# dhamm97/pycsou

Measured on AMD Instinct MI355X. Metric: PDS iters/sec on 4096² TV-deconv; achieved HBM GB/s vs roofline at 1/2/4/8 GPU, higher is better.
Workload: dtype f32

## Files before the change

include/pycsou_hip.h:

```cpp
#ifndef PYCSOU_HIP_H
#define PYCSOU_HIP_H

#include <stdint.h>
#include <hip/hip_runtime_api.h>

#ifdef __cplusplus
extern "C" {
#endif

enum { PCS_F32 = 0, PCS_F64 = 1 };
enum { PCS_OK = 0, PCS_EINVAL = -1, PCS_ELAUNCH = -2, PCS_EUNSUPPORTED = -3 };
enum { PCS_FORWARD = 0, PCS_BACKWARD = 1, PCS_CENTERED = 2 };
enum { PCS_H_L1 = 0, PCS_H_L21 = 1 };
enum { PCS_G_NULL = 0, PCS_G_NONNEG = 1, PCS_G_SEGMENT = 2 };
enum { PCS_F_NULL = 0, PCS_F_DENOISE = 1, PCS_F_SEPCONV = 2, PCS_F_GRADBUF = 3, PCS_F_CONV2D = 4, PCS_F_CONV0 = 5 };
enum { PCS_K_GRAD_FORWARD = 0, PCS_K_GRAD_BACKWARD = 1, PCS_K_GRAD_CENTERED = 2, PCS_K_LAPLACIAN = 3 };

int pcs_abi_version(void);


int pcs_deriv1_fwd(int dtype, const void* x, void* out, int ndim, const int64_t* dims, int axis, double step,
                   int kind, int edge, hipStream_t stream);
int pcs_deriv1_adj(int dtype, const void* y, void* out, int ndim, const int64_t* dims, int axis, double step,
                   int kind, int edge, hipStream_t stream);
// ... 127 lines not shown
  PCS_PATH_SMARCH_NX = 6,
  PCS_PATH_NM64 = 7,
  PCS_PATH_CONV2D = 8
};
int pcs_pds2d_path(const pcs_pds2d_args* a);
int pcs_pds2d_ntaps_len(int half);

int pcs_pds2d_halo_x(int half);
int64_t pcs_pds2d_nblocks(const pcs_pds2d_args* a);
int64_t pcs_pds2d_ws_bytes(const pcs_pds2d_args* a);
int pcs_pds2d_step(const pcs_pds2d_args* a, hipStream_t stream);
int64_t pcs_pds2d_nblocks_bands(const pcs_pds2d_args* a, int64_t ra0, int64_t rb0, int64_t ra1, int64_t rb1);
int pcs_pds2d_step_bands(const pcs_pds2d_args* a, int64_t ra0, int64_t rb0, int64_t ra1, int64_t rb1,
                         hipStream_t stream);
int pcs_pds2d_run(const pcs_pds2d_args* a, int64_t n, hipStream_t stream);

typedef struct {
  int dtype, kkind, fkind, hkind, gkind, edge;
  int64_t n0, n1;
  double tau, sigma, rho, lam, step0, step1, w0, w1, seg_a, seg_b;
  const void* x; void* xn; const void* z; void* zn; const void* g;
  double* partials;
  void* ctrl;
  double* hist;
  void* ws;
} pcs_pds2d_stencil_args;
int64_t pcs_pds2d_stencil_nblocks(const pcs_pds2d_stencil_args* a);
int64_t pcs_pds2d_stencil_ws_bytes(const pcs_pds2d_stencil_args* a);
int pcs_pds2d_stencil_step(const pcs_pds2d_stencil_args* a, hipStream_t stream);
int pcs_pds2d_stencil_run(const pcs_pds2d_stencil_args* a, int64_t n, hipStream_t stream);
// ... 97 lines not shown
```

pycsou_amd/_lib.py:

```python

import ctypes
import os

import torch

_HERE = os.path.dirname(os.path.abspath(__file__))
LIB_PATH = os.environ.get('PCS_LIB_PATH') or os.path.join(_HERE, 'lib', 'libpycsou_hip.so')

PCS_F32, PCS_F64 = 0, 1
PCS_FORWARD, PCS_BACKWARD, PCS_CENTERED = 0, 1, 2
PCS_H_L1, PCS_H_L21 = 0, 1
PCS_K_GRAD_FORWARD, PCS_K_GRAD_BACKWARD, PCS_K_GRAD_CENTERED, PCS_K_LAPLACIAN = 0, 1, 2, 3
PCS_G_NULL, PCS_G_NONNEG, PCS_G_SEGMENT = 0, 1, 2
PCS_APGD_G_L1 = 3
PCS_F_NULL, PCS_F_DENOISE, PCS_F_SEPCONV, PCS_F_GRADBUF, PCS_F_CONV2D, PCS_F_CONV0 = 0, 1, 2, 3, 4, 5
PCS_M_NONE, PCS_M_L1LOSS = 0, 1
(PCS_PATH_TILE, PCS_PATH_MARCH, PCS_PATH_NMARCH, PCS_PATH_PT, PCS_PATH_SMARCH, PCS_PATH_SMARCH_NX, PCS_PATH_NM64,
 PCS_PATH_CONV2D) = range(1, 9)
PCS_PATH_FUSED_NORMAL = (PCS_PATH_NMARCH, PCS_PATH_NM64)
KINDS = {'forward': PCS_FORWARD, 'backward': PCS_BACKWARD, 'centered': PCS_CENTERED}

_c_int, _c_i64, _c_dbl, _vp = ctypes.c_int, ctypes.c_int64, ctypes.c_double, ctypes.c_void_p
_pi64 = ctypes.POINTER(ctypes.c_int64)
_pdbl = ctypes.POINTER(ctypes.c_double)
# ... 98 lines not shown
    'pcs_apgd_step': (_c_int, [_c_int, _vp, _vp, _vp, _vp, _vp, _c_i64, _c_dbl, _c_dbl, _c_int, _c_dbl, _c_dbl,
                                _c_dbl, _vp, _vp, _vp]),
    'pcs_pds2d_halo_x': (_c_int, [_c_int]),
    'pcs_pds2d_ntaps_len': (_c_int, [_c_int]),
    'pcs_pds2d_nblocks': (_c_i64, [ctypes.POINTER(PdsArgs)]),
    'pcs_pds2d_ws_bytes': (_c_i64, [ctypes.POINTER(PdsArgs)]),
    'pcs_pds2d_step': (_c_int, [ctypes.POINTER(PdsArgs), _vp]),
    'pcs_fftconv2d_grid': (_c_i64, [_c_i64, _c_int]),
    'pcs_fftconv2d_create': (_c_int, [_c_int, _c_i64, _c_i64, _pdbl, _c_int, _c_int, _c_int, _c_int,
                                      ctypes.POINTER(_vp)]),
    'pcs_fftconv2d_apply': (_c_int, [_vp, _vp, _vp, _c_int, _vp, _c_dbl, _vp]),
    'pcs_fftconv2d_destroy': (_c_int, [_vp]),
    'pcs_pds2d_supported': (_c_int, [ctypes.POINTER(PdsArgs)]),
    'pcs_pds2d_path': (_c_int, [ctypes.POINTER(PdsArgs)]),
    'pcs_pds2d_run': (_c_int, [ctypes.POINTER(PdsArgs), _c_i64, _vp]),
    'pcs_pds2d_stencil_nblocks': (_c_i64, [ctypes.POINTER(StencilArgs)]),
    'pcs_pds2d_stencil_ws_bytes': (_c_i64, [ctypes.POINTER(StencilArgs)]),
    'pcs_pds2d_stencil_step': (_c_int, [ctypes.POINTER(StencilArgs), _vp]),
    'pcs_pds2d_stencil_run': (_c_int, [ctypes.POINTER(StencilArgs), _c_i64, _vp]),
    'pcs_pds2d_nblocks_bands': (_c_i64, [ctypes.POINTER(PdsArgs), _c_i64, _c_i64, _c_i64, _c_i64]),
    'pcs_pds2d_step_bands': (_c_int, [ctypes.POINTER(PdsArgs), _c_i64, _c_i64, _c_i64, _c_i64, _vp]),
    'pcs_comm_available': (_c_int, []),
    'pcs_comm_id_bytes': (_c_int, []),
    'pcs_comm_unique_id': (_c_int, [_vp]),
    'pcs_comm_init': (_c_int, [_vp, _c_int, _c_int, ctypes.POINTER(_vp)]),
    'pcs_comm_destroy': (_c_int, [_vp]),
    'pcs_allgather_f64': (_c_int, [_vp, _c_int, _vp, _vp, _c_i64, _vp]),
    'pcs_halo_exchange': (_c_int, [_vp, _c_int, _c_int, ctypes.POINTER(HaloSet), _vp]),
    'pcs_slab2d_create': (_c_int, [ctypes.POINTER(Slab2DDesc), _vp, ctypes.POINTER(_vp)]),
    'pcs_slab2d_overlapped': (_c_int, [_vp]),
# ... 86 lines not shown
```

pycsou_amd/csrc/pds.hip:

```cpp
#include "pds_host.hpp"
#include "pds_pt.hpp"

namespace pcs {

__global__ void k_ctrl_init(Ctrl* c, int min_iter, int max_iter, double thr, int has_dual, int hist_len) {
  c->it = 0;
  c->min_iter = min_iter;
  c->max_iter = max_iter;
  c->thr = thr;
  c->has_dual = has_dual;
  c->hist_len = hist_len;
  c->pend = c->pad1 = 0;
  const double inf = __builtin_huge_val();
  c->stopped = !((0 <= min_iter) || (0 <= max_iter && inf > thr));
}

constexpr int kRedThreads = 1024;

__device__ __forceinline__ void sum_partials(const double* __restrict__ part, int64_t np, double (&v)[4]) {
  const double4* p4 = reinterpret_cast<const double4*>(part);
  double4 a[4];
#pragma unroll
  for (int u = 0; u < 4; ++u) a[u] = make_double4(0.0, 0.0, 0.0, 0.0);
  for (int64_t i = threadIdx.x; i < np; i += 4 * kRedThreads) {
// ... 114 lines not shown
                                             : (a->halo_z > a->halo_y ? a->halo_z : a->halo_y);
  if (!(a->n0 < (1LL << 30) && (a->rows + 2 * hmax) * a->n1 * 4 <= (1LL << 30))) return false;
  MarchPlan p;
  return pt_plan(a, full_bands(a), &p);
}

template <int FK, int HK>
static int launch_pt(const pcs_pds2d_args* a, RowBands rb, hipStream_t st) {
  MarchPlan p;
  if (!pt_plan(a, rb, &p)) return PCS_EINVAL;
  if (p.ntasks == 0) return PCS_OK;
  const Slab s64 = make_slab(a);
  const Slab32 s{(int)s64.n0, (int)s64.n1, (int)s64.row0, (int)s64.rows, s64.hx, s64.hy, s64.hz, s64.vec};
  const Params<float> P = make_params<float>(a);
  const float* g = FK == PCS_F_DENOISE ? (const float*)a->y : FK == PCS_F_GRADBUF ? (const float*)a->gbuf : nullptr;
  k_pds2d_pt<FK, HK><<<(unsigned)p.ntasks + fin_extra(a), 256, 0, st>>>((const float*)a->x, (float*)a->xn, (const float*)a->z,
                                                         (float*)a->zn, g, s, P, a->gkind, a->partials,
                                                         (Ctrl*)a->ctrl, a->hist, a->ws, red_out(a), p.tiles_x, p.bd,
                                                         p.ntasks);
  return launch_status();
}

static int64_t bands_nblocks(const pcs_pds2d_args* a, RowBands rb);

template <int FK>
static int launch_pt(const pcs_pds2d_args* a, RowBands rb, hipStream_t st) {
  return a->hkind == PCS_H_L21 ? launch_pt<FK, PCS_H_L21>(a, rb, st) : launch_pt<FK, PCS_H_L1>(a, rb, st);
}

static int pds2d_bands(const pcs_pds2d_args* a, RowBands rb, hipStream_t st) {
  if (use_nm64(a)) return launch_nmarch64(a, rb, st);
  if (use_smarch(a)) return a->dtype == PCS_F64 ? sm_launch<double>(a, rb, st) : sm_launch<float>(a, rb, st);
  if (use_march(a)) return launch_march(a, rb, st);
// ... 190 lines not shown

int pcs_pds2d_step(const pcs_pds2d_args* a, hipStream_t st) {
  int rc = check_args(a);
  if (rc != PCS_OK) return rc;
  if (a->fkind == PCS_F_CONV2D) {
    rc = conv2d_prepass(a, st);
    if (rc != PCS_OK) return rc;
    const pcs_pds2d_args b = step_args(a);
    return pcs_pds2d_step(&b, st);
  }
  if (a->dtype == PCS_F32) return pds2d<float>(a, st);
  if (a->dtype == PCS_F64) return pds2d<double>(a, st);
  return PCS_EINVAL;
}

int pcs_pds2d_run(const pcs_pds2d_args* a, int64_t n, hipStream_t st) {
  if (!a || n < 0 || !a->hist) return PCS_EINVAL;
  pcs_pds2d_args b = *a;
  for (int64_t i = 0; i < n; ++i) {
    if (i % 2) {
      b.x = a->xn, b.xn = const_cast<void*>(a->x), b.z = a->zn, b.zn = const_cast<void*>(a->z);
      b.zm = a->zmn, b.zmn = const_cast<void*>(a->zm);
      if (a->fin_partials) b.partials = const_cast<double*>(a->fin_partials), b.fin_partials = a->partials;
    } else {
      b.x = a->x, b.xn = a->xn, b.z = a->z, b.zn = a->zn;
      b.zm = a->zm, b.zmn = a->zmn;
      b.partials = a->partials, b.fin_partials = a->fin_partials;
    }
    const int rc = pcs_pds2d_step(&b, st);
    if (rc != PCS_OK) return rc;
  }
  return PCS_OK;
}

int64_t pcs_ctrl_bytes(void) { return 64; }

#ifdef PCS_STAMPS
int pcs_debug_stamps(void* host, int64_t bytes) {
  return hipMemcpyFromSymbol(host, HIP_SYMBOL(g_pcs_stamps), (size_t)bytes, 0, hipMemcpyDeviceToHost) == hipSuccess
             ? 0
             : PCS_ELAUNCH;
}
#endif

int pcs_ctrl_init2(void* ctrl, int min_iter, int max_iter, double thr, int has_dual, int hist_len, hipStream_t st) {
// ... 42 lines not shown
```

pycsou_amd/csrc/pds_ctrl.hpp:

```cpp
#pragma once

#include "common.hpp"

namespace pcs {

struct Ctrl {
  int32_t it, stopped, min_iter, max_iter, has_dual, hist_len;
  int32_t pend;
  int32_t pad1;
  double thr;
  double pad2;
};
static_assert(sizeof(Ctrl) == 48, "ctrl layout");

__device__ __forceinline__ void finalize_from(const double* v, Ctrl* c, double* hist) {
  const int it = c->it;
  const double inf = __builtin_huge_val();
  const double rp = (v[1] == 0.0) ? inf : sqrt(v[0]) / sqrt(v[1]);
  const double rd = (v[3] == 0.0) ? inf : sqrt(v[2]) / sqrt(v[3]);
  if (2 * it + 1 < c->hist_len) {
    hist[2 * it] = rp;
    hist[2 * it + 1] = rd;
  }
  const int nx = it + 1;
// ... 36 lines not shown
__device__ __forceinline__ bool stop_deferred(const RedOut& ro) { return PCS_DEFER_STOP && ro.sums == nullptr; }
__device__ __forceinline__ int stop_flag_early(const Ctrl* ctrl, const RedOut& ro) {
  return stop_deferred(ro) && ctrl != nullptr ? ctrl->stopped : 0;
}

__device__ __forceinline__ bool stop_requested(const Ctrl* ctrl, const RedOut& ro, int* flag) {
  if (ctrl == nullptr) return false;
  if (ro.sums == nullptr) return ctrl->stopped != 0;
  if (threadIdx.x == 0) flag[0] = __hip_atomic_load(&ctrl->stopped, __ATOMIC_RELAXED, __HIP_MEMORY_SCOPE_AGENT);
  __syncthreads();
  return flag[0] != 0;
}

constexpr int kFinBlocks = 8;
constexpr int kFinLanes = 256;
__device__ __forceinline__ int fin_shift(const RedOut& ro) { return ro.fin != nullptr ? kFinBlocks : 0; }

__device__ __forceinline__ void finalize_pending(const double* __restrict__ prev, int64_t nb, Ctrl* c, double* hist,
                                                 bool mark, double* red, int* flag) {
  const int tid = threadIdx.x;
  if (tid == 0) flag[0] = c->pend && !c->stopped;
  __syncthreads();
  if (flag[0]) {
    double v[4] = {0.0, 0.0, 0.0, 0.0};
    if (tid < kFinLanes) {
      for (int64_t j = tid; j < nb; j += kFinLanes) {
#pragma unroll
        for (int k = 0; k < 4; ++k) v[k] += prev[j * 4 + k];
      }
    }
    block_sum<4>(v, red);
    if (tid == 0) finalize_from(v, c, hist);
  }
  if (tid == 0) c->pend = mark ? 1 : 0;
}

__device__ __forceinline__ bool fin_slot(const RedOut& ro, int64_t nblocks, Ctrl* ctrl, double* hist, double* red,
                                         int* flag) {
  if (ro.fin == nullptr || blockIdx.x >= kFinBlocks) return false;
  if (blockIdx.x == 0) finalize_pending(ro.fin, nblocks, ctrl, hist, true, red, flag);
  return true;
}

#ifndef PCS_RED_ABL
#define PCS_RED_ABL 0
#endif
__device__ __forceinline__ void reduce_and_finalize(const double (&part)[4], double* __restrict__ partials,
                                                    int64_t nblocks, void* ws, Ctrl* ctrl, double* hist, int* flag,
                                                    RedOut ro = RedOut{nullptr, nullptr, 0, nullptr}) {
  if (PCS_RED_ABL & 1) return;
  const int tid = threadIdx.x;
  const int64_t b = blockIdx.x;
  const int64_t ngr = red_groups(nblocks);
  double* gsum = reinterpret_cast<double*>(ws);
  unsigned* cnt = reinterpret_cast<unsigned*>(gsum + ngr * 4);
// ... 85 lines not shown
```

pycsou_amd/csrc/pds_host.hpp:

```cpp
#pragma once

#include "pds_march.hpp"
#include "pds_nmarch.hpp"
#include "pds_smarch.hpp"

namespace pcs {

template <typename T>
struct Tile {
  static constexpr int TH = 31;
  static constexpr int NT = 256;
};
template <>
struct Tile<double> {
  static constexpr int TH = 15;
  static constexpr int NT = 256;
};

static int tier_for(int half) {
  if (half <= 3) return 3;
  if (half <= 7) return 7;
  if (half <= 11) return 11;
  if (half <= 15) return 15;
  return -1;
// ... 16 lines not shown
  P.rho = (T)a->rho;
  P.omr = (T)(1.0 - a->rho);
  const double t_h = (1.0 / a->sigma) * a->lam;
  P.t_h = (T)t_h;
  P.inv_t_h = (T)(1.0 / t_h);
  P.lam = (T)a->lam;
  P.inv_step0 = (T)(1.0 / a->step0);
  P.inv_step1 = (T)(1.0 / a->step1);
  P.unit0 = a->step0 == 1.0;
  P.unit1 = a->step1 == 1.0;
  P.seg_a = (T)a->seg_a;
  P.seg_b = (T)a->seg_b;
  return P;
}

static RedOut red_out(const pcs_pds2d_args* a) {
  return a->hist ? RedOut{nullptr, nullptr, 0, a->fin_partials}
                 : RedOut{a->sums_out, a->pre_partials, (int)a->n_pre, nullptr};
}
static unsigned fin_extra(const pcs_pds2d_args* a) {
  return a->hist && a->fin_partials ? (unsigned)kFinBlocks : 0u;
}

constexpr int kMarchNT = 256;
constexpr int kNMarchNT = 256;

struct MarchPlan {
  int tiles_x;
  Bands bd;
  int ntasks;
  StripSplit sp{-1, 0, 0, 0, {0, 0, 0}, Bands{16, 0, 0, 0, 0, 0}};
};

struct RowBands {
  int64_t ra0, rb0, ra1, rb1;
};
static RowBands full_bands(const pcs_pds2d_args* a) { return RowBands{0, a->rows, a->rows, a->rows}; }

static void plan_bands(RowBands rb, int TS, int tiles_x, int slots, int min_steps, MarchPlan* p) {
  if (rb.rb0 == rb.ra0) rb = RowBands{rb.ra1, rb.rb1, rb.rb1, rb.rb1};
  const int64_t L0 = rb.rb0 - rb.ra0, L1 = rb.rb1 - rb.ra1;
  const int64_t steps = (L0 + TS - 1) / TS + (L1 + TS - 1) / TS;
  const int64_t bands = (L0 > 0) + (L1 > 0);
  int64_t nseg = slots / tiles_x;
  const int64_t max_seg = (steps + min_steps - 1) / min_steps;
  nseg = nseg > max_seg ? max_seg : nseg;
  nseg = nseg < bands ? bands : nseg;
  nseg = nseg < 1 ? 1 : nseg;
  const int64_t seg_len = ((steps + nseg - 1) / nseg) * TS;
  const int64_t n0 = (L0 + seg_len - 1) / seg_len, n1 = (L1 + seg_len - 1) / seg_len;
  p->tiles_x = tiles_x;
  p->bd = Bands{(int)seg_len, (int)n0, (int)rb.ra0, (int)rb.rb0, (int)rb.ra1, (int)rb.rb1};
  p->ntasks = (int)(tiles_x * (n0 + n1));
}
// ... 156 lines not shown
```

pycsou_amd/csrc/pds_nm.hip:

```cpp
#include "pds_host.hpp"

namespace pcs {

template <int H>
static int march_slots() {
  static int slots = 0;
  if (slots == 0) {
    int dev = 0, cus = 0, nb = 0;
    if (hipGetDevice(&dev) != hipSuccess || hipDeviceGetAttribute(&cus, hipDeviceAttributeMultiprocessorCount, dev) !=
                                                hipSuccess || cus < 1)
      cus = 256;
    if (hipOccupancyMaxActiveBlocksPerMultiprocessor(&nb, k_pds2d_march<float, H, PCS_H_L21, kMarchNT>, kMarchNT,
                                                     0) != hipSuccess ||
        nb < 1)
      nb = 3;
    (void)hipGetLastError();
    slots = cus * nb;
  }
  return slots;
}

template <int H>
static int nmarch_slots(bool gen) {
  static int slots_f = 0, slots_g = 0;
// ... 21 lines not shown

int march_slots_h(int H) { return H == 3 ? march_slots<3>() : march_slots<7>(); }
int nmarch_slots_h(int H, bool gen) { return H == 3 ? nmarch_slots<3>(gen) : nmarch_slots<7>(gen); }

template <int H, int HK>
static int launch_march_k(const pcs_pds2d_args* a, RowBands rb, hipStream_t st) {
  MarchPlan p;
  if (!march_plan<H>(a, rb, &p)) return PCS_EINVAL;
  if (p.ntasks == 0) return PCS_OK;
  const Slab s64 = make_slab(a);
  const Slab32 s{(int)s64.n0, (int)s64.n1, (int)s64.row0, (int)s64.rows, s64.hx, s64.hy, s64.hz, s64.vec};
  const Params<float> P = make_params<float>(a);
  if (use_nmarch(a) && a->kkind != PCS_K_GRAD_FORWARD) {
    auto kern = a->kkind == PCS_K_GRAD_BACKWARD ? k_pds2d_nmarch_gen<float, H, HK, kNMarchNT, PCS_BACKWARD>
                                                : k_pds2d_nmarch_gen<float, H, HK, kNMarchNT, PCS_CENTERED>;
    kern<<<(unsigned)p.ntasks + fin_extra(a), kNMarchNT, 0, st>>>((const float*)a->x, (float*)a->xn, (const float*)a->z, (float*)a->zn,
                                                   (const float*)a->cty, (const float*)a->ntaps, s, P, a->gkind,
                                                   a->edge, a->partials, (Ctrl*)a->ctrl, a->hist, a->ws, red_out(a),
                                                   p.tiles_x, p.bd, p.ntasks);
    return launch_status();
  }
  if (use_nmarch(a)) {
    k_pds2d_nmarch<float, H, HK, kNMarchNT><<<(unsigned)p.ntasks + fin_extra(a), kNMarchNT, 0, st>>>(
        (const float*)a->x, (float*)a->xn, (const float*)a->z, (float*)a->zn, (const float*)a->cty,
        (const float*)a->ntaps, s, P, a->gkind, a->partials, (Ctrl*)a->ctrl, a->hist, a->ws, red_out(a), p.tiles_x,
        p.bd, p.ntasks);
    return launch_status();
  }
  if (a->kkind != PCS_K_GRAD_FORWARD) return PCS_EUNSUPPORTED;
  k_pds2d_march<float, H, HK, kMarchNT><<<(unsigned)p.ntasks + fin_extra(a), kMarchNT, 0, st>>>(
      (const float*)a->x, (float*)a->xn, (const float*)a->z, (float*)a->zn, (const float*)a->y,
      (const float*)a->taps0, (const float*)a->taps1, a->half, s, P, a->gkind, a->partials, (Ctrl*)a->ctrl, a->hist,
      a->ws, red_out(a), p.tiles_x, p.bd, p.ntasks);
  return launch_status();
}

template <int H>
static int launch_march_k(const pcs_pds2d_args* a, RowBands rb, hipStream_t st) {
  return a->hkind == PCS_H_L21 ? launch_march_k<H, PCS_H_L21>(a, rb, st) : launch_march_k<H, PCS_H_L1>(a, rb, st);
}

int launch_march(const pcs_pds2d_args* a, RowBands rb, hipStream_t st) {
  return tier_for(a->half) == 3 ? launch_march_k<3>(a, rb, st) : launch_march_k<7>(a, rb, st);
}

}
```

pycsou_amd/csrc/pds_nm64.hip:

```cpp
#include "pds_host.hpp"

namespace pcs {

template <int H>
struct NM64 {
  static constexpr int NT = 512, TS = 32, TO = 60, CW = 64, CC = CW / 2;
  static constexpr int NQ = 4 * H + 1;
  static constexpr int XOFF = 16, XW = CW + 2 * XOFF, XCH = XW / 2;
  static constexpr int XRING = 48, XP = XW + 2;
  static constexpr int TRING = TS + 4 * H, TMIR = 4 * H + 1, TP = CW + 2;
  static constexpr int URING = TS + 2, UP = CW + 2;
  static constexpr int ZR = TS + 2, ZCH = CC + 2;
  static constexpr int ZSL = ZR * ZCH, ZINS = (ZSL + 63) / 64;
  static constexpr int NW = 64 + 32 * H;
  static constexpr int NXL = (TS * XCH + NT - 1) / NT;
  static constexpr int O_X = 0, O_T = O_X + XRING * XP, O_U = O_T + (TRING + TMIR) * TP, O_Z = O_U + URING * UP,
                       O_W = O_Z + 2 * (ZINS * 64 * 2), SZ = O_W + NW;
  static_assert(XRING >= TS + 2 * H, "x ring holds the U rows and the PH rows of a step");
  static_assert(NT == 16 * CC && NT == TS * 16, "one PH item and one PV / U / Z item per thread");
  static __device__ __forceinline__ int xslot(int r) { return (int)((unsigned)(r + XRING * (1 << 20)) % XRING); }
  static __device__ __forceinline__ int tslot(int r) { return (int)((unsigned)(r + TRING * (1 << 20)) % TRING); }
  static __device__ __forceinline__ int uslot(int r) { return (int)((unsigned)(r + URING * (1 << 20)) % URING); }
};

// ... 420 lines not shown
    if (hipOccupancyMaxActiveBlocksPerMultiprocessor(&nb, k_pds2d_nmarch64<7, PCS_H_L21, PCS_CENTERED>, 512,
                                                     NM64<7>::SZ * sizeof(double)) != hipSuccess ||
        nb < 1)
      nb = 1;
    (void)hipGetLastError();
    slots = cus * nb;
    const char* e = getenv("PCS_NM64_SLOTS");
    if (e && atoi(e) > 0) slots = atoi(e);
  }
  return slots;
}

bool nm64_plan(const pcs_pds2d_args* a, RowBands rb, MarchPlan* p) {
  const int tiles_x = (int)((a->n1 + 59) / 60);
  if (tiles_x < 2) return false;
  if (rb.rb0 == rb.ra0) rb = RowBands{rb.ra1, rb.rb1, rb.rb1, rb.rb1};
  const int64_t L0 = rb.rb0 - rb.ra0, L1 = rb.rb1 - rb.ra1;
  const int64_t steps = (L0 + 31) / 32 + (L1 + 31) / 32;
  const int64_t bands = (L0 > 0) + (L1 > 0);
  const int64_t slots = nm64_slots();
  int64_t best = -1, seg_len = 32;
  for (int64_t nseg = bands; nseg <= steps && nseg <= 64; ++nseg) {
    const int64_t len = ((steps + nseg - 1) / nseg) * 32;
    const int64_t n = (L0 + len - 1) / len + (L1 + len - 1) / len;
    const int64_t rounds = (n * tiles_x + slots - 1) / slots;
    const int64_t cost = rounds * (len / 32 + 1);
    if (best < 0 || cost < best) {
      best = cost;
      seg_len = len;
    }
  }
  const int64_t n0s = (L0 + seg_len - 1) / seg_len, n1s = (L1 + seg_len - 1) / seg_len;
  p->tiles_x = tiles_x;
  p->bd = Bands{(int)seg_len, (int)n0s, (int)rb.ra0, (int)rb.rb0, (int)rb.ra1, (int)rb.rb1};
  p->ntasks = (int)(tiles_x * (n0s + n1s));
  return true;
}

template <int H, int HK, int KK>
static int nm64_go(const pcs_pds2d_args* a, const MarchPlan& p, hipStream_t st) {
  const Slab s64 = make_slab(a);
  const Slab32 s{(int)s64.n0, (int)s64.n1, (int)s64.row0, (int)s64.rows, s64.hx, s64.hy, s64.hz, s64.vec};
  const Params<double> P = make_params<double>(a);
  nm64_attr<H, HK, KK>();
  k_pds2d_nmarch64<H, HK, KK><<<(unsigned)p.ntasks + fin_extra(a), 512, NM64<H>::SZ * sizeof(double), st>>>(
      (const double*)a->x, (double*)a->xn, (const double*)a->z, (double*)a->zn, (const double*)a->cty,
      (const double*)a->ntaps, s, P, a->gkind, a->edge, a->partials, (Ctrl*)a->ctrl, a->hist, a->ws, red_out(a),
      p.tiles_x, p.bd, p.ntasks);
  return launch_status();
}

template <int H, int HK>
static int nm64_k(const pcs_pds2d_args* a, const MarchPlan& p, hipStream_t st) {
  switch (a->kkind) {
    case PCS_K_GRAD_FORWARD: return nm64_go<H, HK, PCS_FORWARD>(a, p, st);
    case PCS_K_GRAD_BACKWARD: return nm64_go<H, HK, PCS_BACKWARD>(a, p, st);
    case PCS_K_GRAD_CENTERED: return nm64_go<H, HK, PCS_CENTERED>(a, p, st);
    default: return PCS_EUNSUPPORTED;
  }
}

int launch_nmarch64(const pcs_pds2d_args* a, RowBands rb, hipStream_t st) {
// ... 10 lines not shown
```

pycsou_amd/csrc/pds_nmarch.hpp:

```cpp
#pragma once
#ifndef PCS_NM_WPE
#define PCS_NM_WPE 3
#endif
#ifndef PCS_NM_PF
#define PCS_NM_PF 2
#endif
#ifndef PCS_NM_EDGE
#define PCS_NM_EDGE 1
#endif
#ifndef PCS_NM_SAUX
#define PCS_NM_SAUX 16
#endif

#include <type_traits>

#include "pds_march.hpp"
#include "stencil.hpp"

namespace pcs {

__device__ __forceinline__ void pcs_fence() {
  asm volatile("" ::: "memory");
  __builtin_amdgcn_sched_barrier(0);
}
// ... 18 lines not shown
  static_assert(N >= 0 && N < 64, "vmcnt");
  __builtin_amdgcn_s_waitcnt((N & 15) | ((N >> 4) << 14) | (7 << 4) | (15 << 8));
}

#ifndef PCS_NM_LAUX
#define PCS_NM_LAUX 0
#endif
template <int AUX>
__device__ __forceinline__ G4<float> bload4a(Rsrc r, uint32_t off) {
  const auto v = __builtin_amdgcn_raw_buffer_load_b128(r, (int)off, 0, AUX);
  return {{__uint_as_float(v[0]), __uint_as_float(v[1]), __uint_as_float(v[2]), __uint_as_float(v[3])}};
}

#ifndef PCS_NM_XEARLY
#define PCS_NM_XEARLY 1
#endif

#ifndef PCS_NM_COOP65
#define PCS_NM_COOP65 1
#endif

__device__ __forceinline__ float row_sum16(float v) {
  v += __int_as_float(__builtin_amdgcn_update_dpp(0, __float_as_int(v), 0x128, 0xf, 0xf, false));
  v += __int_as_float(__builtin_amdgcn_update_dpp(0, __float_as_int(v), 0x124, 0xf, 0xf, false));
  v += __int_as_float(__builtin_amdgcn_update_dpp(0, __float_as_int(v), 0x122, 0xf, 0xf, false));
  v += __int_as_float(__builtin_amdgcn_update_dpp(0, __float_as_int(v), 0x121, 0xf, 0xf, false));
  return v;
}

#ifndef PCS_NM_COLS
// ... 825 lines not shown
  const int stop_raw = stop_flag_early(ctrl, ro);
  const bool stopped = !stop_deferred(ro) && stop_requested(ctrl, ro, flag);
  if (stopped && ro.sums == nullptr) return;

  int task;
  {
    const int bb = (int)blockIdx.x - fin_shift(ro), q = ntasks / 8, r = ntasks % 8, xcd = bb % 8, k = bb / 8;
    task = (xcd < r ? xcd * (q + 1) : r * (q + 1) + (xcd - r) * q) + k;
  }
  const int seg = task / tiles_x, strip = task - seg * tiles_x;
  int s0, s1;
  band_rows(bd, seg, s0, s1);
  const int c0 = strip * M::TW;

  double part[4] = {0.0, 0.0, 0.0, 0.0};
  if (!stopped)
    nmarch_task<T, H, HK, NT, PCS_FORWARD>(x, xn, z, zn, b, tq, s, P, gk, 0, s0, s1, c0, sm, zs0, zs1, part, stop_raw);
  if (stop_raw) return;
  block_sum<4>(part, red);
  publish_partials(part, partials, ntasks, ws, ctrl, hist, flag, ro);
}

template <typename T, int H, int HK, int NT, int KK>
__global__ __launch_bounds__(NT) __attribute__((amdgpu_waves_per_eu(PCS_NM_WPE))) void k_pds2d_nmarch_gen(
    const T* __restrict__ x, T* __restrict__ xn, const T* __restrict__ z, T* __restrict__ zn,
    const T* __restrict__ b, const T* __restrict__ tq, Slab32 s, Params<T> P, int gk, int edge,
    double* __restrict__ partials, Ctrl* ctrl, double* hist, void* ws, RedOut ro, int tiles_x, Bands bd,
    int ntasks) {
  static_assert(KK == PCS_BACKWARD || KK == PCS_CENTERED, "k_pds2d_nmarch is the forward kernel");
  using M = NMarch<H, true>;
  __shared__ __attribute__((aligned(16))) T sm[M::SZ];
  __shared__ __attribute__((aligned(16))) T zs0[4 * M::ZSLOTS];
// ... 27 lines not shown
```

pycsou_amd/csrc/pds_sm_impl.hpp:

```cpp
#pragma once

#include "pds_host.hpp"

namespace pcs {

template <typename T>
int sm_slots() {
  static int slots = 0;
  if (slots == 0) {
    int dev = 0, cus = 0, nb = 0;
    if (hipGetDevice(&dev) != hipSuccess || hipDeviceGetAttribute(&cus, hipDeviceAttributeMultiprocessorCount, dev) !=
                                                hipSuccess || cus < 1)
      cus = 256;
    if (hipOccupancyMaxActiveBlocksPerMultiprocessor(&nb, k_pds2d_smarch<T, PCS_CENTERED, PCS_F_DENOISE, PCS_H_L21>,
                                                     256, 0) != hipSuccess ||
        nb < 1)
      nb = sizeof(T) == 4 ? 3 : 2;
    (void)hipGetLastError();
    slots = cus * (nb < 3 ? nb : 3);
    if (sizeof(T) == 8) slots *= 3;
    const char* e = getenv("PCS_SM_SLOTS");
    if (e && atoi(e) > 0) slots = atoi(e);
  }
  return slots;
// ... 13 lines not shown
template <typename T, int KK, int FK, int HK>
static int launch_smarch(const pcs_pds2d_args* a, RowBands rb, hipStream_t st) {
  MarchPlan p;
  if (!sm_plan(a, rb, &p)) return PCS_EINVAL;
  if (p.ntasks == 0) return PCS_OK;
  const Slab s64 = make_slab(a);
  const Slab32 s{(int)s64.n0, (int)s64.n1, (int)s64.row0, (int)s64.rows, s64.hx, s64.hy, s64.hz, s64.vec};
  const Params<T> P = make_params<T>(a);
  const T* g = FK == PCS_F_DENOISE                       ? (const T*)a->y
               : (FK == PCS_F_GRADBUF || FK == SM_F_NB) ? (const T*)a->gbuf
                                                        : nullptr;
  const T* b = FK == SM_F_NB ? (const T*)a->cty : nullptr;
  if constexpr (FK == SM_F_MASK) g = (const T*)a->ym;
  const T* mi = FK == SM_F_MASK ? (const T*)a->zm : nullptr;
  T* mo = FK == SM_F_MASK ? (T*)a->zmn : nullptr;
  k_pds2d_smarch<T, KK, FK, HK><<<(unsigned)p.ntasks + fin_extra(a), 256, 0, st>>>((const T*)a->x, (T*)a->xn, (const T*)a->z, (T*)a->zn, g, b, mi, mo, s, P,
                                           make_sparams<T>(a), a->gkind, a->partials, (Ctrl*)a->ctrl, a->hist, a->ws,
                                           red_out(a), p.tiles_x, p.bd, p.ntasks, p.sp);
  return launch_status();
}

template <typename T, int KK, int FK>
static int launch_smarch(const pcs_pds2d_args* a, RowBands rb, hipStream_t st) {
  if constexpr (KK == SK_LAP) return launch_smarch<T, KK, FK, PCS_H_L1>(a, rb, st);
  else
    return a->hkind == PCS_H_L21 ? launch_smarch<T, KK, FK, PCS_H_L21>(a, rb, st)
                                 : launch_smarch<T, KK, FK, PCS_H_L1>(a, rb, st);
}

template <typename T, int KK>
static int launch_smarch(const pcs_pds2d_args* a, RowBands rb, hipStream_t st) {
  if (a->fkind == PCS_F_SEPCONV) {
    if ((KK == PCS_FORWARD && sizeof(T) == 4) || rb.ra0 != 0 || rb.rb0 != a->rows) return PCS_EUNSUPPORTED;
// ... 41 lines not shown
```

pycsou_amd/opt/engine.py:

```python

import ctypes
import os

import numpy as np
import torch

from .. import _lib as L
from .. import _ops as O
from ..core.functional import ProxFuncPostComp
from ..core.map import DiffMapComp, DiffMapShifted
from ..func.base import IndicatorFunctional, NullDifferentiableFunctional, NullProximableFunctional
from ..func.penalty import L1Norm, L21Norm, SquaredL2Norm
from ..linop.base import HomothetyMap
from ..linop.conv import Convolve2DOp
from ..linop.diff import GradientOp, LaplacianOp

NATIVE_MIN_PIXELS = int(os.environ.get('PCS_NATIVE_MIN_PIXELS', 1 << 20))


HIST_CHUNK = 4096

DEFER_FIN = os.environ.get('PCS_DEFER_FIN', '1') != '0'


# ... 200 lines not shown
        self.nblocks = int(self.lib.pcs_pds2d_nblocks(ctypes.byref(a)))
        self._alloc_partials(a, dev)
        self.ctrl = torch.zeros(int(self.lib.pcs_ctrl_bytes()) // 8, dtype=torch.float64, device=dev)
        a.ctrl = self.ctrl.data_ptr()
        self.fused_finalize = True
        self.ws = torch.zeros(int(self.lib.pcs_pds2d_ws_bytes(ctypes.byref(a))) // 8 + 2, dtype=torch.float64,
                              device=dev)
        a.ws = self.ws.data_ptr()
        self.graph = None
        self.hist = None
        self.ctrl_host = torch.zeros(2, dtype=torch.int32).pin_memory()
        self.native = fk != L.PCS_F_GRADBUF and self.N >= NATIVE_MIN_PIXELS

    def _alloc_partials(self, a, dev):
        self.defer = DEFER_FIN and isinstance(a, L.PdsArgs)
        nb4 = self.nblocks * 4
        self.partials = torch.empty((2 if self.defer else 1) * nb4, dtype=torch.float64, device=dev)
        self.part_halves = [self.partials[:nb4], self.partials[nb4:]] if self.defer else [self.partials]
        a.partials = self.partials.data_ptr()
        if self.defer:
            a.fin_partials = self.part_halves[1].data_ptr()

    def _bind(self, a, p):
        a.x, a.xn = self.X[p].data_ptr(), self.X[1 - p].data_ptr()
        a.z, a.zn = self.Z[p].data_ptr(), self.Z[1 - p].data_ptr()
        if getattr(self, 'defer', False):
            a.partials, a.fin_partials = self.part_halves[p].data_ptr(), self.part_halves[1 - p].data_ptr()

    def _flush(self, next_p, hist):
        if getattr(self, 'defer', False):
            L.check(self.lib.pcs_pds_finalize_pending(L.ptr(self.part_halves[1 - next_p]), self.nblocks,
                                                      L.ptr(self.ctrl), L.ptr(hist), L.stream()),
                    'pcs_pds_finalize_pending')

    def _step_call(self, st):
        L.check(self.lib.pcs_pds2d_step(ctypes.byref(self.args), st), 'pcs_pds2d_step')

    def _run_call(self, n):
        L.check(self.lib.pcs_pds2d_run(ctypes.byref(self.args), int(n), L.stream()), 'pcs_pds2d_run')

    def _iteration(self, p, hist):
        a, lib, st = self.args, self.lib, L.stream()
        if self.fkind == L.PCS_F_GRADBUF:
            self._grad_conv(p, st)
        self._bind(a, p)
        a.hist = hist.data_ptr() if self.fused_finalize else None
# ... 42 lines not shown

    def replay(self):
        if self.native:
            self._chunk_native(self.hist)
        else:
            self.graph.replay()

    def advance_fixed(self, n):
        p = getattr(self, '_fixed_p', 0)
        if self.native:
            a = self.args
            self._bind(a, p)
            a.hist = self.hist.data_ptr()
            self._run_call(int(n))
            self._fixed_p = p ^ (int(n) & 1)
            self._flush(self._fixed_p, self.hist)
            return
        while n >= self.chunk and p == 0:
            self.graph.replay()
            n -= self.chunk
        for _ in range(n):
            self._iteration(p, self.hist)
            p ^= 1
        self._fixed_p = p
        self._flush(p, self.hist)

    def time_iteration_kernels(self, n):
        a, lib = self.args, self.lib
        st = torch.cuda.current_stream()
        n = min(n, (self.hist.numel() - 2) // 2 - 1)
        L.check(lib.pcs_ctrl_init2(L.ptr(self.ctrl), n + 1, n + 1, -1.0, 1, int(self.hist.numel()), L.stream()),
# ... 82 lines not shown
                ev = torch.cuda.Event()
                self.ctrl_host.copy_(self.ctrl.view(torch.int32)[:2], non_blocking=True)
                ev.record()
                pending.append(ev)
                if len(pending) >= 2:
                    pending.pop(0).synchronize()
                    if int(self.ctrl_host[1]) != 0:
                        break
        else:
            for k in range(n_chunks):
                self.hist = grow_hist(self.hist, self.ctrl, (k + 1) * self.chunk + 1, total)
                self._chunk(self.hist)
                if int(self.ctrl.view(torch.int32)[1].item()) != 0:
                    break
        hist = self.hist
        self._flush(0, hist)
        torch.cuda.synchronize()
        c = self.ctrl.view(torch.int32)[:2].cpu().numpy()
        n = int(c[0])
        h = hist[:2 * n].cpu().numpy().reshape(n, 2) if n > 0 else np.zeros((0, 2))
        return n, self.X[n % 2], self.Z[n % 2], h


class PDS2DStencilEngine(PDS2DEngine):

    def __init__(self, spec, dtype, tau, sigma, rho, x0, z0, chunk=32, use_graph=True):
        self.lib = L.gpu()
        self.spec = spec
        self.dtype = dtype
        n0, n1 = spec['shape']
        self.N = N = n0 * n1
# ... 227 lines not shown
```

Measured before the change: 9216.

## Split each PDS run iteration into alternating top/bottom row-band launches

In the native multi-iteration run, each step can now be issued as two row-band launches (top half and bottom half), with the band order alternating between iterations. The aim is that the band written last in one iteration is read first in the next while it is still cache-resident. Plan selection is gated by an env var (PCS_RUN_BANDS) and working-set size thresholds, and the deferred-finalize partial-sum bookkeeping is extended so the first launch finalizes using the combined block count. It also adds a G_NULL specialization branch in the nmarch forward task.

```diff
diff --git a/include/pycsou_hip.h b/include/pycsou_hip.h
--- a/include/pycsou_hip.h
+++ b/include/pycsou_hip.h
@@ -165,6 +165,8 @@
 int pcs_pds2d_step_bands(const pcs_pds2d_args* a, int64_t ra0, int64_t rb0, int64_t ra1, int64_t rb1,
                          hipStream_t stream);
 int pcs_pds2d_run(const pcs_pds2d_args* a, int64_t n, hipStream_t stream);
+int64_t pcs_pds2d_run_nblocks(const pcs_pds2d_args* a, int mode);
+int pcs_pds2d_run_plan(const pcs_pds2d_args* a, int mode, int64_t i, int64_t* out);
 
 typedef struct {
   int dtype, kkind, fkind, hkind, gkind, edge;
diff --git a/pycsou_amd/_lib.py b/pycsou_amd/_lib.py
--- a/pycsou_amd/_lib.py
+++ b/pycsou_amd/_lib.py
@@ -136,6 +136,8 @@
     'pcs_pds2d_supported': (_c_int, [ctypes.POINTER(PdsArgs)]),
     'pcs_pds2d_path': (_c_int, [ctypes.POINTER(PdsArgs)]),
     'pcs_pds2d_run': (_c_int, [ctypes.POINTER(PdsArgs), _c_i64, _vp]),
+    'pcs_pds2d_run_nblocks': (_c_i64, [ctypes.POINTER(PdsArgs), _c_int]),
+    'pcs_pds2d_run_plan': (_c_int, [ctypes.POINTER(PdsArgs), _c_int, _c_i64, ctypes.POINTER(_c_i64)]),
     'pcs_pds2d_stencil_nblocks': (_c_i64, [ctypes.POINTER(StencilArgs)]),
     'pcs_pds2d_stencil_ws_bytes': (_c_i64, [ctypes.POINTER(StencilArgs)]),
     'pcs_pds2d_stencil_step': (_c_int, [ctypes.POINTER(StencilArgs), _vp]),
diff --git a/pycsou_amd/csrc/pds.hip b/pycsou_amd/csrc/pds.hip
--- a/pycsou_amd/csrc/pds.hip
+++ b/pycsou_amd/csrc/pds.hip
@@ -1,3 +1,5 @@
+#include <cstring>
+
 #include "pds_host.hpp"
 #include "pds_pt.hpp"
 
@@ -152,9 +154,9 @@
   const Slab32 s{(int)s64.n0, (int)s64.n1, (int)s64.row0, (int)s64.rows, s64.hx, s64.hy, s64.hz, s64.vec};
   const Params<float> P = make_params<float>(a);
   const float* g = FK == PCS_F_DENOISE ? (const float*)a->y : FK == PCS_F_GRADBUF ? (const float*)a->gbuf : nullptr;
-  k_pds2d_pt<FK, HK><<<(unsigned)p.ntasks + fin_extra(a), 256, 0, st>>>((const float*)a->x, (float*)a->xn, (const float*)a->z,
+  k_pds2d_pt<FK, HK><<<(unsigned)p.ntasks + fin_extra(a, p.fin_n), 256, 0, st>>>((const float*)a->x, (float*)a->xn, (const float*)a->z,
                                                          (float*)a->zn, g, s, P, a->gkind, a->partials,
-                                                         (Ctrl*)a->ctrl, a->hist, a->ws, red_out(a), p.tiles_x, p.bd,
+                                                         (Ctrl*)a->ctrl, a->hist, a->ws, red_out(a, p.fin_n), p.tiles_x, p.bd,
                                                          p.ntasks);
   return launch_status();
 }
@@ -375,8 +377,54 @@
   return PCS_EINVAL;
 }
 
+constexpr int64_t kPairSetMin = 336LL << 20;
+constexpr int64_t kPairHalfMax = 224LL << 20;
+
+struct RunPlan {
+  bool paired;
+  int64_t m, nT, nB;
+};
+
+static RunPlan run_plan(const pcs_pds2d_args* a, int mode) {
+  RunPlan r{false, 0, 0, 0};
+  if (mode < 0) {
+    const char* e = getenv("PCS_RUN_BANDS");
+    mode = e == nullptr || *e == '\0' ? 0 : strcmp(e, "auto") == 0 ? 2 : atoi(e);
+  }
+  if (mode <= 0 || mode > 2 || check_args(a) != PCS_OK) return r;
+  if (a->rows != a->n0 || a->mkind != PCS_M_NONE || a->fkind == PCS_F_CONV2D) return r;
+  if (use_smarch(a) && a->fkind == PCS_F_SEPCONV) return r;
+  if (!(use_nm64(a) || use_smarch(a) || use_march(a) || (a->kkind == PCS_K_GRAD_FORWARD && use_pt(a)))) return r;
+  const int64_t m = (a->rows / 2 + 8) / 16 * 16;
+  if (m <= 0 || m >= a->rows) return r;
+  if (mode != 1) {
+    const int64_t row = 7 * a->n1 * (a->dtype == PCS_F64 ? 8 : 4), big = m > a->rows - m ? m : a->rows - m;
+    if (a->rows * row < kPairSetMin || big * row > kPairHalfMax) return r;
+  }
+  const int64_t nT = bands_nblocks(a, RowBands{0, m, m, m}), nB = bands_nblocks(a, RowBands{m, a->rows, a->rows, a->rows});
+  if (nT < 1 || nB < 1) return r;
+  return RunPlan{true, m, nT, nB};
+}
+
+int64_t pcs_pds2d_run_nblocks(const pcs_pds2d_args* a, int mode) {
+  if (!a) return -1;
+  const RunPlan r = run_plan(a, mode);
+  return r.paired ? r.nT + r.nB : pcs_pds2d_nblocks(a);
+}
+
+int pcs_pds2d_run_plan(const pcs_pds2d_args* a, int mode, int64_t i, int64_t* out) {
+  if (!a || !out || i < 0) return PCS_EINVAL;
+  const RunPlan r = run_plan(a, mode);
+  const bool top_first = i % 2 == 0;
+  out[0] = r.paired, out[1] = r.m, out[2] = r.nT, out[3] = r.nB;
+  out[4] = r.paired && !top_first ? r.m : 0;
+  out[5] = r.paired && top_first ? r.m : a->rows;
+  return PCS_OK;
+}
+
 int pcs_pds2d_run(const pcs_pds2d_args* a, int64_t n, hipStream_t st) {
   if (!a || n < 0 || !a->hist) return PCS_EINVAL;
+  const RunPlan rp = a->fin_partials ? run_plan(a, -1) : RunPlan{false, 0, 0, 0};
   pcs_pds2d_args b = *a;
   for (int64_t i = 0; i < n; ++i) {
     if (i % 2) {
@@ -388,8 +436,19 @@
       b.zm = a->zm, b.zmn = a->zmn;
       b.partials = a->partials, b.fin_partials = a->fin_partials;
     }
-    const int rc = pcs_pds2d_step(&b, st);
-    if (rc != PCS_OK) return rc;
+    if (!rp.paired) {
+      const int rc = pcs_pds2d_step(&b, st);
+      if (rc != PCS_OK) return rc;
+      continue;
+    }
+    double* const part = b.partials;
+    for (int k = 0; k < 2; ++k) {
+      const bool top = (k == 0) == (i % 2 == 0);
+      const int64_t lo = top ? 0 : rp.m, hi = top ? rp.m : a->rows;
+      b.partials = part + (top ? 0 : rp.nT * 4);
+      const int rc = pds2d_bands(&b, RowBands{lo, hi, hi, hi, k == 0 ? rp.nT + rp.nB : -1}, st);
+      if (rc != PCS_OK) return rc;
+    }
   }
   return PCS_OK;
 }
diff --git a/pycsou_amd/csrc/pds_ctrl.hpp b/pycsou_amd/csrc/pds_ctrl.hpp
--- a/pycsou_amd/csrc/pds_ctrl.hpp
+++ b/pycsou_amd/csrc/pds_ctrl.hpp
@@ -74,7 +74,8 @@
 
 constexpr int kFinBlocks = 8;
 constexpr int kFinLanes = 256;
-__device__ __forceinline__ int fin_shift(const RedOut& ro) { return ro.fin != nullptr ? kFinBlocks : 0; }
+__device__ __forceinline__ bool fin_slots(const RedOut& ro) { return ro.fin != nullptr && ro.npre >= 0; }
+__device__ __forceinline__ int fin_shift(const RedOut& ro) { return fin_slots(ro) ? kFinBlocks : 0; }
 
 __device__ __forceinline__ void finalize_pending(const double* __restrict__ prev, int64_t nb, Ctrl* c, double* hist,
                                                  bool mark, double* red, int* flag) {
@@ -97,8 +98,8 @@
 
 __device__ __forceinline__ bool fin_slot(const RedOut& ro, int64_t nblocks, Ctrl* ctrl, double* hist, double* red,
                                          int* flag) {
-  if (ro.fin == nullptr || blockIdx.x >= kFinBlocks) return false;
-  if (blockIdx.x == 0) finalize_pending(ro.fin, nblocks, ctrl, hist, true, red, flag);
+  if (!fin_slots(ro) || blockIdx.x >= kFinBlocks) return false;
+  if (blockIdx.x == 0) finalize_pending(ro.fin, ro.npre > 0 ? ro.npre : nblocks, ctrl, hist, true, red, flag);
   return true;
 }
 
diff --git a/pycsou_amd/csrc/pds_host.hpp b/pycsou_amd/csrc/pds_host.hpp
--- a/pycsou_amd/csrc/pds_host.hpp
+++ b/pycsou_amd/csrc/pds_host.hpp
@@ -54,12 +54,12 @@
   return P;
 }
 
-static RedOut red_out(const pcs_pds2d_args* a) {
-  return a->hist ? RedOut{nullptr, nullptr, 0, a->fin_partials}
+static RedOut red_out(const pcs_pds2d_args* a, int64_t fin_n = 0) {
+  return a->hist ? RedOut{nullptr, nullptr, a->fin_partials ? (int)fin_n : 0, a->fin_partials}
                  : RedOut{a->sums_out, a->pre_partials, (int)a->n_pre, nullptr};
 }
-static unsigned fin_extra(const pcs_pds2d_args* a) {
-  return a->hist && a->fin_partials ? (unsigned)kFinBlocks : 0u;
+static unsigned fin_extra(const pcs_pds2d_args* a, int64_t fin_n = 0) {
+  return a->hist && a->fin_partials && fin_n >= 0 ? (unsigned)kFinBlocks : 0u;
 }
 
 constexpr int kMarchNT = 256;
@@ -69,15 +69,18 @@
   int tiles_x;
   Bands bd;
   int ntasks;
+  int64_t fin_n = 0;
   StripSplit sp{-1, 0, 0, 0, {0, 0, 0}, Bands{16, 0, 0, 0, 0, 0}};
 };
 
 struct RowBands {
   int64_t ra0, rb0, ra1, rb1;
+  int64_t fin_n = 0;
 };
 static RowBands full_bands(const pcs_pds2d_args* a) { return RowBands{0, a->rows, a->rows, a->rows}; }
 
 static void plan_bands(RowBands rb, int TS, int tiles_x, int slots, int min_steps, MarchPlan* p) {
+  p->fin_n = rb.fin_n;
   if (rb.rb0 == rb.ra0) rb = RowBands{rb.ra1, rb.rb1, rb.rb1, rb.rb1};
   const int64_t L0 = rb.rb0 - rb.ra0, L1 = rb.rb1 - rb.ra1;
   const int64_t steps = (L0 + TS - 1) / TS + (L1 + TS - 1) / TS;
diff --git a/pycsou_amd/csrc/pds_nm.hip b/pycsou_amd/csrc/pds_nm.hip
--- a/pycsou_amd/csrc/pds_nm.hip
+++ b/pycsou_amd/csrc/pds_nm.hip
@@ -59,24 +59,24 @@
   if (use_nmarch(a) && a->kkind != PCS_K_GRAD_FORWARD) {
     auto kern = a->kkind == PCS_K_GRAD_BACKWARD ? k_pds2d_nmarch_gen<float, H, HK, kNMarchNT, PCS_BACKWARD>
                                                 : k_pds2d_nmarch_gen<float, H, HK, kNMarchNT, PCS_CENTERED>;
-    kern<<<(unsigned)p.ntasks + fin_extra(a), kNMarchNT, 0, st>>>((const float*)a->x, (float*)a->xn, (const float*)a->z, (float*)a->zn,
+    kern<<<(unsigned)p.ntasks + fin_extra(a, p.fin_n), kNMarchNT, 0, st>>>((const float*)a->x, (float*)a->xn, (const float*)a->z, (float*)a->zn,
                                                    (const float*)a->cty, (const float*)a->ntaps, s, P, a->gkind,
-                                                   a->edge, a->partials, (Ctrl*)a->ctrl, a->hist, a->ws, red_out(a),
+                                                   a->edge, a->partials, (Ctrl*)a->ctrl, a->hist, a->ws, red_out(a, p.fin_n),
                                                    p.tiles_x, p.bd, p.ntasks);
     return launch_status();
   }
   if (use_nmarch(a)) {
-    k_pds2d_nmarch<float, H, HK, kNMarchNT><<<(unsigned)p.ntasks + fin_extra(a), kNMarchNT, 0, st>>>(
+    k_pds2d_nmarch<float, H, HK, kNMarchNT><<<(unsigned)p.ntasks + fin_extra(a, p.fin_n), kNMarchNT, 0, st>>>(
         (const float*)a->x, (float*)a->xn, (const float*)a->z, (float*)a->zn, (const float*)a->cty,
-        (const float*)a->ntaps, s, P, a->gkind, a->partials, (Ctrl*)a->ctrl, a->hist, a->ws, red_out(a), p.tiles_x,
+        (const float*)a->ntaps, s, P, a->gkind, a->partials, (Ctrl*)a->ctrl, a->hist, a->ws, red_out(a, p.fin_n), p.tiles_x,
         p.bd, p.ntasks);
     return launch_status();
   }
   if (a->kkind != PCS_K_GRAD_FORWARD) return PCS_EUNSUPPORTED;
-  k_pds2d_march<float, H, HK, kMarchNT><<<(unsigned)p.ntasks + fin_extra(a), kMarchNT, 0, st>>>(
+  k_pds2d_march<float, H, HK, kMarchNT><<<(unsigned)p.ntasks + fin_extra(a, p.fin_n), kMarchNT, 0, st>>>(
       (const float*)a->x, (float*)a->xn, (const float*)a->z, (float*)a->zn, (const float*)a->y,
       (const float*)a->taps0, (const float*)a->taps1, a->half, s, P, a->gkind, a->partials, (Ctrl*)a->ctrl, a->hist,
-      a->ws, red_out(a), p.tiles_x, p.bd, p.ntasks);
+      a->ws, red_out(a, p.fin_n), p.tiles_x, p.bd, p.ntasks);
   return launch_status();
 }
 
diff --git a/pycsou_amd/csrc/pds_nm64.hip b/pycsou_amd/csrc/pds_nm64.hip
--- a/pycsou_amd/csrc/pds_nm64.hip
+++ b/pycsou_amd/csrc/pds_nm64.hip
@@ -458,6 +458,7 @@
 bool nm64_plan(const pcs_pds2d_args* a, RowBands rb, MarchPlan* p) {
   const int tiles_x = (int)((a->n1 + 59) / 60);
   if (tiles_x < 2) return false;
+  p->fin_n = rb.fin_n;
   if (rb.rb0 == rb.ra0) rb = RowBands{rb.ra1, rb.rb1, rb.rb1, rb.rb1};
   const int64_t L0 = rb.rb0 - rb.ra0, L1 = rb.rb1 - rb.ra1;
   const int64_t steps = (L0 + 31) / 32 + (L1 + 31) / 32;
@@ -487,9 +488,9 @@
   const Slab32 s{(int)s64.n0, (int)s64.n1, (int)s64.row0, (int)s64.rows, s64.hx, s64.hy, s64.hz, s64.vec};
   const Params<double> P = make_params<double>(a);
   nm64_attr<H, HK, KK>();
-  k_pds2d_nmarch64<H, HK, KK><<<(unsigned)p.ntasks + fin_extra(a), 512, NM64<H>::SZ * sizeof(double), st>>>(
+  k_pds2d_nmarch64<H, HK, KK><<<(unsigned)p.ntasks + fin_extra(a, p.fin_n), 512, NM64<H>::SZ * sizeof(double), st>>>(
       (const double*)a->x, (double*)a->xn, (const double*)a->z, (double*)a->zn, (const double*)a->cty,
-      (const double*)a->ntaps, s, P, a->gkind, a->edge, a->partials, (Ctrl*)a->ctrl, a->hist, a->ws, red_out(a),
+      (const double*)a->ntaps, s, P, a->gkind, a->edge, a->partials, (Ctrl*)a->ctrl, a->hist, a->ws, red_out(a, p.fin_n),
       p.tiles_x, p.bd, p.ntasks);
   return launch_status();
 }
diff --git a/pycsou_amd/csrc/pds_nmarch.hpp b/pycsou_amd/csrc/pds_nmarch.hpp
--- a/pycsou_amd/csrc/pds_nmarch.hpp
+++ b/pycsou_amd/csrc/pds_nmarch.hpp
@@ -56,6 +56,10 @@
 
 #ifndef PCS_NM_XEARLY
 #define PCS_NM_XEARLY 1
+#endif
+
+#ifndef PCS_NM_GKSPLIT
+#define PCS_NM_GKSPLIT 1
 #endif
 
 #ifndef PCS_NM_COOP65
@@ -911,8 +915,13 @@
   const int c0 = strip * M::TW;
 
   double part[4] = {0.0, 0.0, 0.0, 0.0};
-  if (!stopped)
-    nmarch_task<T, H, HK, NT, PCS_FORWARD>(x, xn, z, zn, b, tq, s, P, gk, 0, s0, s1, c0, sm, zs0, zs1, part, stop_raw);
+  if (!stopped) {
+    if (PCS_NM_GKSPLIT && gk == PCS_G_NULL)
+      nmarch_task<T, H, HK, NT, PCS_FORWARD>(x, xn, z, zn, b, tq, s, P, PCS_G_NULL, 0, s0, s1, c0, sm, zs0, zs1, part,
+                                             stop_raw);
+    else
+      nmarch_task<T, H, HK, NT, PCS_FORWARD>(x, xn, z, zn, b, tq, s, P, gk, 0, s0, s1, c0, sm, zs0, zs1, part, stop_raw);
+  }
   if (stop_raw) return;
   block_sum<4>(part, red);
   publish_partials(part, partials, ntasks, ws, ctrl, hist, flag, ro);
diff --git a/pycsou_amd/csrc/pds_sm_impl.hpp b/pycsou_amd/csrc/pds_sm_impl.hpp
--- a/pycsou_amd/csrc/pds_sm_impl.hpp
+++ b/pycsou_amd/csrc/pds_sm_impl.hpp
@@ -51,9 +51,9 @@
   if constexpr (FK == SM_F_MASK) g = (const T*)a->ym;
   const T* mi = FK == SM_F_MASK ? (const T*)a->zm : nullptr;
   T* mo = FK == SM_F_MASK ? (T*)a->zmn : nullptr;
-  k_pds2d_smarch<T, KK, FK, HK><<<(unsigned)p.ntasks + fin_extra(a), 256, 0, st>>>((const T*)a->x, (T*)a->xn, (const T*)a->z, (T*)a->zn, g, b, mi, mo, s, P,
+  k_pds2d_smarch<T, KK, FK, HK><<<(unsigned)p.ntasks + fin_extra(a, p.fin_n), 256, 0, st>>>((const T*)a->x, (T*)a->xn, (const T*)a->z, (T*)a->zn, g, b, mi, mo, s, P,
                                            make_sparams<T>(a), a->gkind, a->partials, (Ctrl*)a->ctrl, a->hist, a->ws,
-                                           red_out(a), p.tiles_x, p.bd, p.ntasks, p.sp);
+                                           red_out(a, p.fin_n), p.tiles_x, p.bd, p.ntasks, p.sp);
   return launch_status();
 }
 
diff --git a/pycsou_amd/opt/engine.py b/pycsou_amd/opt/engine.py
--- a/pycsou_amd/opt/engine.py
+++ b/pycsou_amd/opt/engine.py
@@ -238,7 +238,14 @@
 
     def _alloc_partials(self, a, dev):
         self.defer = DEFER_FIN and isinstance(a, L.PdsArgs)
-        nb4 = self.nblocks * 4
+        self.run_nblocks = cap = self.nblocks
+        if self.defer:
+            a.x, a.xn = self.X[0].data_ptr(), self.X[1].data_ptr()
+            a.z, a.zn = self.Z[0].data_ptr(), self.Z[1].data_ptr()
+            a.partials = a.x
+            self.run_nblocks = int(self.lib.pcs_pds2d_run_nblocks(ctypes.byref(a), -1))
+            cap = max(cap, self.run_nblocks, int(self.lib.pcs_pds2d_run_nblocks(ctypes.byref(a), 1)))
+        nb4 = cap * 4
         self.partials = torch.empty((2 if self.defer else 1) * nb4, dtype=torch.float64, device=dev)
         self.part_halves = [self.partials[:nb4], self.partials[nb4:]] if self.defer else [self.partials]
         a.partials = self.partials.data_ptr()
@@ -251,9 +258,10 @@
         if getattr(self, 'defer', False):
             a.partials, a.fin_partials = self.part_halves[p].data_ptr(), self.part_halves[1 - p].data_ptr()
 
-    def _flush(self, next_p, hist):
+    def _flush(self, next_p, hist, run=False):
         if getattr(self, 'defer', False):
-            L.check(self.lib.pcs_pds_finalize_pending(L.ptr(self.part_halves[1 - next_p]), self.nblocks,
+            L.check(self.lib.pcs_pds_finalize_pending(L.ptr(self.part_halves[1 - next_p]),
+                                                      self.run_nblocks if run else self.nblocks,
                                                       L.ptr(self.ctrl), L.ptr(hist), L.stream()),
                     'pcs_pds_finalize_pending')
 
@@ -326,7 +334,7 @@
             a.hist = self.hist.data_ptr()
             self._run_call(int(n))
             self._fixed_p = p ^ (int(n) & 1)
-            self._flush(self._fixed_p, self.hist)
+            self._flush(self._fixed_p, self.hist, run=True)
             return
         while n >= self.chunk and p == 0:
             self.graph.replay()
@@ -439,7 +447,7 @@
                 if int(self.ctrl.view(torch.int32)[1].item()) != 0:
                     break
         hist = self.hist
-        self._flush(0, hist)
+        self._flush(0, hist, run=self.native)
         torch.cuda.synchronize()
         c = self.ctrl.view(torch.int32)[:2].cpu().numpy()
         n = int(c[0])
```

After: 9427, median of 6. 2.3% higher.
